# hsiehScalAR/KNODE-Cosserat

Hardware: AMD Instinct MI355X
Metric: rod-steps/sec (N=100 segments, batch=1024) (higher is better)
Workload: dtype f64

## Files before the change

### knode-cosserat_amd/csrc/kr_mso_impl.hpp

```cpp
#pragma once
#include "kr_ms_impl.hpp"

namespace kr {

constexpr int MSO_B0 = 7 + 17 * (MS_P - 1);
#ifndef KR_MSO_LAG
#define KR_MSO_LAG 1
#endif
constexpr int MSO_LAG = KR_MSO_LAG;
static_assert(MSO_B0 + MS_P <= WAVE, "the verifying lanes must fit beside the forward-difference lanes");

template <typename T, int HS>
__host__ __device__ inline size_t mso_lds_elems(int N) {
  return ms_lds_elems<T, HS>(N, true, false) + 80;
}

__device__ __forceinline__ void wave_sync_lds() {
  __builtin_amdgcn_fence(__ATOMIC_ACQ_REL, "wavefront");
  __builtin_amdgcn_wave_barrier();
}

#define KR_LDS __attribute__((address_space(3)))
template <typename T, int NV>
__device__ __forceinline__ void lds_load_vec(const T* src, T (&v)[NV]) {
  using V = typename Vec16<T>::type;
  constexpr int n = Vec16<T>::n;
  static_assert(NV % n == 0, "vector load needs a multiple of 16 bytes");
  const KR_LDS V* s = (const KR_LDS V*)src;
#pragma unroll
  for (int c = 0; c < NV / n; ++c) {
    const V x = s[c];
#pragma unroll
    for (int e = 0; e < n; ++e) v[c * n + e] = x[e];
  }
}
template <typename T, int NV>
__device__ __forceinline__ void lds_store_vec(T* dst, const T (&v)[NV]) {
  using V = typename Vec16<T>::type;
  constexpr int n = Vec16<T>::n;
  static_assert(NV % n == 0, "vector store needs a multiple of 16 bytes");
  KR_LDS V* d = (KR_LDS V*)dst;
#pragma unroll
  for (int c = 0; c < NV / n; ++c) {
    V x;
#pragma unroll
    for (int e = 0; e < n; ++e) x[e] = v[c * n + e];
    d[c] = x;
  }
}

template <typename U>
__device__ __forceinline__ U own_sgpr(U v) {
  asm volatile("" : "+s"(v));
  return v;
}

template <typename U>
__device__ __forceinline__ U* own_sgpr_global(U* p) {
  uintptr_t v = (uintptr_t)p;
  asm volatile("" : "+s"(v));
  return (U*)(__attribute__((address_space(1))) U*)v;
}

#ifdef KR_MS_STAMPS
struct MsoStats { unsigned long long total = 0, sweeps = 0, merged = 0, quick = 0, chord = 0, rejects = 0, retries = 0, rebuilds = 0, t_sweep = 0, t_alg = 0, t_pred = 0, t_verdict = 0, t_cond = 0, t_fin = 0, t_upd = 0, t_v1 = 0, t_v2 = 0, t_c1 = 0, t_c2 = 0, t_copy = 0; };
#endif

template <typename T, bool DIAG, int HS, int OCC = 1, typename PSRC = RodConst<T>>
__global__ __launch_bounds__(WAVE * MS_WPB, OCC) void mso_sim_kernel(const PSRC Pa, const SimArgs<T> A) {
  extern __shared__ __attribute__((aligned(16))) unsigned char smem_raw[];
  const int N = rod_src_N<T>(Pa);
  const int lane = threadIdx.x & (WAVE - 1);
  const int wv = threadIdx.x / WAVE;
  const int64_t rod = (int64_t)blockIdx.x * MS_WPB + wv;
  if (rod >= A.B) return;
  const auto& Pc = rod_src_row<T>(Pa, rod);
  const size_t rod_elems = (size_t)N * KR_SLOTS;
  T* const a_states = own_sgpr_global(A.states);
  const int64_t a_slot_elems = own_sgpr(A.slot_elems);
  const int a_ring = own_sgpr(A.ring);
  T* const a_tip = own_sgpr_global(A.tip);
  int32_t* const a_status = own_sgpr_global(A.status);
  const int a_residual_test = own_sgpr(A.residual_test), a_predictor = own_sgpr(A.predictor);
  const T hc1 = own_sgpr(A.hc1), hc2 = own_sgpr(A.hc2);
  const int T_steps = own_sgpr((int)A.T_steps);
  const MsLds<T> L = ms_carve<T, HS>(reinterpret_cast<T*>(smem_raw) + (size_t)wv * mso_lds_elems<T, HS>(N), N, true, false);
  T* const Es = L.Es;
  T* const XB = L.XB;
  T* const Tm = L.Tm;
  T* const X0 = L.Xs;
  const ptrdiff_t X_d = (L.c12 + (size_t)N * 12) - L.Xs;
  int xsel = 0;
  T* Xs = X0;
  T* XsB = X0 + X_d;
  T* const EsB = Es + MSO_B0 * MS_YP;
  const MsRole R = ms_role(lane, N);
  const int iv = R.iv, col = R.col;
  const bool isA = lane < MSO_B0;
  const bool isB = lane >= MSO_B0 && lane < MSO_B0 + MS_P;
  const int ib = isB ? lane - MSO_B0 : 0;
  const int s_l = isB ? ms_interval_start(ib, R.sbase, R.srem) : R.s_i;
  const int len_l = isB ? R.sbase + (ib < R.srem ? 1 : 0) : R.len_i;
  ms_cold_fill<T>(rod_src_mem<T>(Pa, rod), L.cold, lane);
  wave_sync();

  auto slot_ptr = [&](int slot) -> T* { return a_states + (int64_t)slot * a_slot_elems + rod * rod_elems; };
  auto state_ptr = [&](int k) -> T* { return slot_ptr(a_ring ? k % 3 : k); };
  T* const lead0 = L.c12;
  const ptrdiff_t lead_d = L.hist - L.c12;
  auto lead_of = [&](int t) -> T* { return lead0 + (ptrdiff_t)(t & 1) * lead_d; };
  auto rebuild = [&](int t) {
    const T* cur = state_ptr(t);
    const T* prv = t > 0 ? state_ptr(t - 1) : (A.prev_init ? A.prev_init + rod * rod_elems : cur);
    T* const lc = lead_of(t);
    T* const lp = lead_of(t - 1);
    for (int j = lane; j < N; j += WAVE) {
      T cv[12], pv[12];
      load_hist_vec<T, 12>(cur + (size_t)j * KR_SLOTS, cv);
      load_hist_vec<T, 12>(prv + (size_t)j * KR_SLOTS, pv);
      lds_store_vec<T, 12>(lc + (size_t)j * 12, cv);
      lds_store_vec<T, 12>(lp + (size_t)j * 12, pv);
    }
    wave_sync();
  };
  const T* ctl = A.ctl + rod * A.T_steps * 4;
  auto load_fc = [&](int t) -> V3<T> {
    V3<T> tf{T(0), T(0), T(0)};
#pragma unroll
    for (int k = 0; k < 4; ++k) {
      const T tt = ctl[(size_t)t * 4 + k];
      tf.x += tt * L.cold[CD_TDIRS + k * 3 + 0];
      tf.y += tt * L.cold[CD_TDIRS + k * 3 + 1];
      tf.z += tt * L.cold[CD_TDIRS + k * 3 + 2];
    }
    return {L.cold[CD_RHOAG] + tf.x, L.cold[CD_RHOAG + 1] + tf.y, L.cold[CD_RHOAG + 2] + tf.z};
  };

  const T* s0 = state_ptr(0);
  const T* sp0 = A.prev_init ? A.prev_init + rod * rod_elems : s0;
  MsPred<T> Q;
  double* img = A.pred_io ? A.pred_io + (size_t)rod * MS_PRED_ROWS * WAVE : nullptr;
  if (img && A.pred_load) ms_pred_load<T>(Q, img, lane);
  else ms_pred_init<T>(Q, lane, R, s0, sp0, A.prev_init != nullptr, a_predictor);
  V3<T> vlast, ulast;
  {
    const T* cl = s0 + (size_t)(N - 1) * KR_SLOTS;
    vlast = {cl[SL_V], cl[SL_V + 1], cl[SL_V + 2]};
    ulast = {cl[SL_U], cl[SL_U + 1], cl[SL_U + 2]};
  }
  const T tol = own_sgpr(A.tol), tolA = own_sgpr(A.tolA), fd_eps = own_sgpr(A.fd_eps);
  const int maxit = own_sgpr(A.maxit);
  T kappa = Q.kappa;
  T Gguess = lane < 6 ? A.G[rod * 6 + lane] : T(0);
  MsStamps stamps;
#ifdef KR_MS_STAMPS
  MsoStats st;
  unsigned long long t_begin, tq;
  KR_STAMP(t_begin);
  tq = t_begin;
#endif

  rebuild(0);

  int tA = 0;
  int rsA = 0;
  bool merged = false;
  int it = 0;
  int order = Q.next_order;
  bool retried = false;
  T dn_prev = T(-1);
  bool have_fac = false, below = false;
  float amp = -1.f;
  T dnB = T(-1);
  float ampB = -1.f;
  bool belowB = false;
  int itB = 0, orderB = 0;
  bool pred_skip = false;
  bool reverify = false;
  int resume_at = T_steps;
  T Xreg[MS_P - 1][2];
#pragma unroll
  for (int g = 0; g < MS_P - 1; ++g) Xreg[g][0] = Xreg[g][1] = T(0);
  V3<T> fcA = load_fc(0), fcB = fcA;
  V3<T> fcN = load_fc(T_steps > 1 ? 1 : 0);
  static_assert(DIAG, "the in-sweep history record assumes diagonal material matrices");
  T hk_a[3], hk_b[3], hk_c[3];
#pragma unroll
  for (int c = 0; c < 3; ++c) {
    hk_a[c] = L.cold[CD_KSEI + 4 * c] * L.cold[CD_KSEV + c];
    hk_b[c] = -L.cold[CD_KSEI + 4 * c] * L.cold[CD_BSE + 4 * c];
    hk_c[c] = -L.cold[CD_KBTI + 4 * c] * L.cold[CD_BBT + 4 * c];
  }

  ms_pred_guess<T>(Q, order, lane, L.cold, Xs);
  wave_sync_lds();
  if (order <= 0 && lane < 6) Xs[0 * MS_YP + 7 + lane] = Gguess;
  wave_sync_lds();

  struct Upd { T updP, updG, xsP, xsG, xsY[MS_P - 1]; };

  while (true) {
    const bool runA = tA < T_steps;
    const int tB = tA - 1;
    T yr[19];
    {
      const T* src = isB ? XsB + ib * MS_YP : Xs + iv * MS_YP;
#pragma unroll
      for (int q = 0; q < 19; ++q) yr[q] = src[q];
    }
    const T hstep = (isA && col > 0) ? fd_eps * fmax(fabs(Xs[iv * MS_YP + (R.comp > 0 ? R.comp : 3)]), T(1)) : T(1);
    int comp = R.comp;
    asm volatile("" : "+v"(comp));
#pragma unroll
    for (int q = 3; q < 19; ++q) yr[q] += q == comp ? hstep : T(0);
    RodState<T> y = rows_to_state(yr);
    const V3<T> fc = isB ? fcB : fcA;
    const int lag = (isA && merged) ? MSO_LAG : 0;
    const bool act = isB ? merged : (isA && runA);
    const int trips = R.lmax + ((merged && runA) ? MSO_LAG : 0);
    T* const out_rod = slot_ptr(rsA);
    auto point_of = [&](int k) -> int {
      const int kk = k - lag;
      return s_l + (kk < 0 ? 0 : (kk < len_l ? kk : len_l - 1));
    };
    const T* const lead_n = lead_of(isB ? tB : tA);
    const T* const lead_o = lead_of(isB ? tB + 1 : tB);
    auto hist_older = [&](const T (&lb)[12], T (&pb)[12]) __attribute__((always_inline)) {
#pragma unroll
      for (int c = 0; c < 12; ++c) pb[c] = hc2 * lb[c];
    };
    auto hist_newest = [&](const T (&la)[12], const T (&pb)[12]) __attribute__((always_inline)) -> RodHist<T> {
      T raw[12];
#pragma unroll
      for (int c = 0; c < 12; ++c) raw[c] = fma(hc1, la[c], pb[c]);
      RodHist<T> h;
      h.qh = {raw[0], raw[1], raw[2]};
      h.wh = {raw[3], raw[4], raw[5]};
      h.vh = {raw[6], raw[7], raw[8]};
      h.uh = {raw[9], raw[10], raw[11]};
      h.av = {hk_b[0] * raw[6] + hk_a[0], hk_b[1] * raw[7] + hk_a[1], hk_b[2] * raw[8] + hk_a[2]};
      h.au = {hk_c[0] * raw[9], hk_c[1] * raw[10], hk_c[2] * raw[11]};
      return h;
    };
    auto hist_form = [&](const T (&la)[12], const T (&lb)[12]) __attribute__((always_inline)) -> RodHist<T> {
      T pb[12];
      hist_older(lb, pb);
      return hist_newest(la, pb);
    };
    auto hist_at = [&](int j) __attribute__((always_inline)) -> RodHist<T> {
      T la[12], lb[12];
      lds_load_vec<T, 12>(lead_n + (size_t)j * 12, la);
      lds_load_vec<T, 12>(lead_o + (size_t)j * 12, lb);
      return hist_form(la, lb);
    };
    RodHist<T> hst = hist_at(point_of(0));
    if (!merged) {
      auto fd_point = [&](int j, T dsl) __attribute__((always_inline)) {
        RodState<T> k1;
        V3<T> v, u;
        ode_eval<T, DIAG>(Pc, y, hst, fc, k1, v, u);
        hst = hist_at(j + 1);
        y = state_axpy(y, dsl, k1);
      };
#pragma unroll 2
      for (int t = 0; t < R.sbase; ++t) fd_point(R.s_i + t, Pc.ds);
      if (R.srem) fd_point(R.s_i + (R.len_i > R.sbase ? R.sbase : R.sbase - 1), R.len_i > R.sbase ? Pc.ds : T(0));
    } else {
      const bool lean = a_ring && tB + 4 <= T_steps;
      T* const lead_w = lead_of(tB + 1);
      auto trip = [&](int k, auto full_tag, auto lean_tag) __attribute__((always_inline)) {
        constexpr bool FULL = decltype(full_tag)::value;
        constexpr bool LEAN = decltype(lean_tag)::value;
        const int kk = k - lag;
        const bool live = FULL ? act : (act && kk >= 0 && kk < len_l);
        const int j = FULL ? s_l + kk : point_of(k);
        const int eo = j * 12;
        const int en = FULL ? eo + 12 : point_of(k + 1) * 12;
        T la[12], lb[12], pb[12];
        if constexpr (MSO_LAG >= 2) {
          lds_load_vec<T, 12>(lead_n + en, la);
          lds_load_vec<T, 12>(lead_o + en, lb);
        } else {
          lds_load_vec<T, 12>(lead_o + en, lb);
#ifdef KR_MSO_PROBE_EARLY_READS
          if constexpr (FULL) lds_load_vec<T, 12>(lead_n + en, la);
#endif
        }
        RodState<T> k1;
        V3<T> v, u;
        ode_eval<T, DIAG>(Pc, y, hst, fc, k1, v, u);
        if constexpr (MSO_LAG >= 2) {
          hst = hist_form(la, lb);
          asm volatile("" : "+v"(hst.qh.x), "+v"(hst.qh.y), "+v"(hst.qh.z), "+v"(hst.wh.x), "+v"(hst.wh.y), "+v"(hst.wh.z));
          asm volatile("" : "+v"(hst.vh.x), "+v"(hst.vh.y), "+v"(hst.vh.z), "+v"(hst.uh.x), "+v"(hst.uh.y), "+v"(hst.uh.z));
          asm volatile("" : "+v"(hst.av.x), "+v"(hst.av.y), "+v"(hst.av.z), "+v"(hst.au.x), "+v"(hst.au.y), "+v"(hst.au.z));
        } else {
          hist_older(lb, pb);
          asm volatile("" : "+v"(pb[0]), "+v"(pb[1]), "+v"(pb[2]), "+v"(pb[3]), "+v"(pb[4]), "+v"(pb[5]), "+v"(pb[6]), "+v"(pb[7]),
                            "+v"(pb[8]), "+v"(pb[9]), "+v"(pb[10]), "+v"(pb[11]));
        }
        if (isB && live) {
          T rec[KR_SLOTS];
          record_from(y, v, u, rec);
          T lead[12];
#pragma unroll
          for (int c = 0; c < 12; ++c) lead[c] = rec[c];
          if constexpr (FULL) {
            if constexpr (!LEAN) {
              T rest[KR_SLOTS - 12];
#pragma unroll
              for (int c = 0; c < KR_SLOTS - 12; ++c) rest[c] = rec[12 + c];
              store_vec<T, KR_SLOTS - 12>(out_rod + (size_t)j * KR_SLOTS + 12, rest);
            }
          } else {
            if (!(lean && k >= R.sbase)) store_record(out_rod + (size_t)j * KR_SLOTS, rec);
          }
          lds_store_vec<T, 12>(lead_w + eo, lead);
        }
        if constexpr (MSO_LAG < 2) {
#ifdef KR_MSO_PROBE_EARLY_READS
          if constexpr (!FULL)
#endif
          lds_load_vec<T, 12>(lead_n + en, la);
          if constexpr (OCC == 1) __builtin_amdgcn_sched_barrier(0);
        }
        const T dsl = live ? Pc.ds : T(0);
        y = state_axpy(y, dsl, k1);
        if constexpr (MSO_LAG < 2) {
          asm volatile("" : "+v"(pb[0]), "+v"(pb[1]), "+v"(pb[2]), "+v"(pb[3]), "+v"(pb[4]), "+v"(pb[5]), "+v"(pb[6]), "+v"(pb[7]),
                            "+v"(pb[8]), "+v"(pb[9]), "+v"(pb[10]), "+v"(pb[11]), "+v"(y.p.z), "+v"(y.h3), "+v"(y.n.z), "+v"(y.m.z),
                            "+v"(y.q.z), "+v"(y.w.z));
          hst = hist_newest(la, pb);
        }
      };
      int k = 0;
      for (; k < MSO_LAG && k < trips; ++k) trip(k, std::false_type{}, std::false_type{});
      auto full_trips = [&](auto lean_tag) __attribute__((always_inline)) {
        for (; k + 1 < R.sbase; k += 2) {
          trip(k, std::true_type{}, lean_tag);
          trip(k + 1, std::true_type{}, lean_tag);
        }
        if (k < R.sbase) {
          trip(k, std::true_type{}, lean_tag);
          ++k;
        }
      };
      if (lean) full_trips(std::true_type{});
      else full_trips(std::false_type{});
      for (; k < trips; ++k) trip(k, std::false_type{}, std::false_type{});
    }
#ifdef KR_MS_STAMPS
    KR_STAMP_ADD(st.t_sweep, tq);
    st.sweeps += 1;
    if (merged) st.merged += 1;
#endif

    int ln = lane;
    asm volatile("" : "+v"(ln));
    const int kp = ln & 3;
    const int r = 3 + (ln >> 2);
    const bool plane = ln < 3 * (MS_P - 1);
    const int pi = plane ? ln / 3 : 0;
    const int prow = plane ? ln - 3 * pi : 0;
    const bool glane = ln >= WAVE - 6;
    T er[19];
    state_to_rows(y, er);
    T d[6];
    T updY[MS_P - 1];
    T* dYb = XB;
    float dnf = 0.f;
    bool finite = true;
    Upd U;

    auto finish = [&](const T* X, auto base_slot) -> float {
      T* sp = Tm;
      if (kp == 0) {
#pragma unroll
        for (int g = 1; g < MS_P - 1; ++g) dYb[g * MS_YP + r] = updY[g - 1];
      }
      wave_sync_lds();
      if (plane) {
        const int l0 = pi == 0 ? 0 : 7 + 17 * (pi - 1);
        T s = Es[base_slot(pi) * MS_YP + prow] - X[(pi + 1) * MS_YP + prow];
        T av[16], dv[16];
#pragma unroll
        for (int c = 0; c < 16; ++c) {
          const bool use = pi > 0 || c < 6;
          av[c] = use ? Es[(l0 + 1 + c) * MS_YP + prow] : T(0);
          dv[c] = pi > 0 ? dYb[pi * MS_YP + 3 + c] : T(0);
        }
        __builtin_amdgcn_sched_barrier(0);
        T s2 = T(0);
#pragma unroll
        for (int c = 0; c < 16; c += 2) {
          const T da = pi > 0 ? dv[c] : (c < 6 ? d[c < 6 ? c : 0] : T(0));
          const T db = pi > 0 ? dv[c + 1] : (c + 1 < 6 ? d[c + 1 < 6 ? c + 1 : 0] : T(0));
          s = fma(av[c], da, s);
          s2 = fma(av[c + 1], db, s2);
        }
        sp[pi * 3 + prow] = s + s2;
      }
      wave_sync_lds();
      float nf = 0.f;
      U.updP = T(0); U.updG = T(0); U.xsP = T(0); U.xsG = T(0);
      if (plane) {
        U.xsP = X[(pi + 1) * MS_YP + prow];
#pragma unroll
        for (int i = 0; i < MS_P - 1; ++i) {
          const T t = sp[i * 3 + prow];
          U.updP += i <= pi ? t : T(0);
        }
        nf = update_ratio(U.updP, U.xsP);
      }
      if (glane) {
        const int k = ln - (WAVE - 6);
        U.xsG = X[0 * MS_YP + 7 + k];
        U.updG = k == 0 ? d[0] : k == 1 ? d[1] : k == 2 ? d[2] : k == 3 ? d[3] : k == 4 ? d[4] : d[5];
        nf = fmaxf(nf, update_ratio(U.updG, U.xsG));
      }
#pragma unroll
      for (int g = 1; g < MS_P; ++g) {
        U.xsY[g - 1] = T(0);
        if (((g - 1) & 3) == kp) {
          U.xsY[g - 1] = X[g * MS_YP + r];
          nf = fmaxf(nf, update_ratio(updY[g - 1], U.xsY[g - 1]));
        }
      }
      return wave_max_nonneg(nf);
    };
    auto apply = [&](T* X) {
      if (plane) X[(pi + 1) * MS_YP + prow] = U.xsP + U.updP;
      if (glane) X[0 * MS_YP + 7 + (ln - (WAVE - 6))] = U.xsG + U.updG;
#pragma unroll
      for (int g = 1; g < MS_P; ++g)
        if (((g - 1) & 3) == kp) X[g * MS_YP + r] = U.xsY[g - 1] + updY[g - 1];
    };

    const bool es_stored = merged;
    if (merged) {
      if (isB || (isA && col == 0)) {
#pragma unroll
        for (int q = 0; q < 19; ++q) Es[ln * MS_YP + q] = er[q];
      }
      if (isB) {
        if (ib == MS_P - 1) {
          T rec[KR_SLOTS];
          record_from(y, vlast, ulast, rec);
          store_record(out_rod + (size_t)(N - 1) * KR_SLOTS, rec);
          T lead[12];
#pragma unroll
          for (int c = 0; c < 12; ++c) lead[c] = rec[c];
          lds_store_vec<T, 12>(lead_of(tB + 1) + (size_t)(N - 1) * 12, lead);
          if (a_tip) {
            T* tp = a_tip + (rod * T_steps + tB) * 3;
            tp[0] = y.p.x; tp[1] = y.p.y; tp[2] = y.p.z;
          }
        }
      }
      wave_sync_lds();
#ifdef KR_MS_STAMPS
      unsigned long long tv;
      { KR_STAMP(tv); st.t_v1 += tv - tq; }
#endif
      float rn = 0.f;
      if (ln < 3 * MS_YP) {
        const int g = ln / MS_YP, q = ln - MS_YP * g;
        const T x = XsB[(g + 1) * MS_YP + q];
        rn = update_ratio(EsB[g * MS_YP + q] - x, x);
      } else if (ln < 3 * MS_YP + 6) {
        const int k = ln - 3 * MS_YP;
        const T e = EsB[(MS_P - 1) * MS_YP + 7 + k];
        rn = update_ratio(L.cold[CD_FTIP + k] - e, e);
      }
      rn = wave_max_nonneg(rn);
#ifdef KR_MS_STAMPS
      KR_STAMP_ADD(st.t_v2, tv);
#endif
      const float est = ampB * rn;
      bool accepted = a_residual_test != 0 && ampB > 0.f && T(256) * (T)est <= tol;
      float dnv = est;
#ifdef KR_MS_STAMPS
      if (accepted) st.quick += 1;
#endif
      if (!accepted) {
        T* ach = XB;
        T* rt = XB + 4 * MS_YP;
        dYb = XB + MS_YP * 8;
        T areg[MS_P - 1];
        areg[0] = EsB[0 * MS_YP + r] - XsB[1 * MS_YP + r];
        if (kp == 0) ach[1 * MS_YP + r] = areg[0];
        wave_sync_lds();
#pragma unroll
        for (int g = 1; g < MS_P; ++g) {
          const int l0 = 7 + 17 * (g - 1);
          T av[4], xv[4];
#pragma unroll
          for (int cc = 0; cc < 4; ++cc) {
            av[cc] = Es[(l0 + 1 + 4 * kp + cc) * MS_YP + r];
            xv[cc] = ach[g * MS_YP + 3 + 4 * kp + cc];
          }
          const T e0 = EsB[g * MS_YP + r];
          const T ynext = g < MS_P - 1 ? XsB[(g + 1) * MS_YP + r] : T(0);
          T part = fma(av[0], xv[0], av[1] * xv[1]) + fma(av[2], xv[2], av[3] * xv[3]);
          part += quad_xor<0xB1>(part);
          part += quad_xor<0x4E>(part);
          if (g < MS_P - 1) {
            areg[g] = e0 - ynext + part;
            if (kp == 0) ach[(g + 1) * MS_YP + r] = areg[g];
          } else if (kp == 0 && r >= 7 && r < 13) {
            rt[r - 7] = L.cold[CD_FTIP + (r - 7)] - e0 - part;
          }
          wave_sync_lds();
        }
        {
          T rtv[6];
#pragma unroll
          for (int j = 0; j < 6; ++j) rtv[j] = rt[j];
#pragma unroll
          for (int i = 0; i < 6; ++i) {
            T acc = T(0);
#pragma unroll
            for (int j = 0; j < 6; ++j) acc = fma(L.Ti[i * 6 + j], rtv[j], acc);
            d[i] = acc;
          }
        }
        {
          const T dd0 = kp == 0 ? T(0) : kp == 1 ? d[1] : kp == 2 ? d[3] : d[5];
          const T dd1 = kp == 0 ? d[0] : kp == 1 ? d[2] : kp == 2 ? d[4] : T(0);
#pragma unroll
          for (int g = 1; g < MS_P; ++g) {
            T sx = fma(Xreg[g - 1][1], dd1, Xreg[g - 1][0] * dd0);
            sx += quad_xor<0xB1>(sx);
            sx += quad_xor<0x4E>(sx);
            updY[g - 1] = areg[g - 1] + sx;
          }
        }
        dnv = finish(XsB, [](int g) { return MSO_B0 + g; });
        accepted = dnv <= 3.0e38f && (T)dnv <= T(0.5) * tol;
#ifdef KR_MS_STAMPS
        st.chord += 1;
#endif
      }
      if (accepted) {
        {
          const T* const lt = lead_of(tB + 1);
          for (int j = ln; j < N; j += WAVE) {
            T lv[12];
            lds_load_vec<T, 12>(lt + (size_t)j * 12, lv);
            store_vec<T, 12>(out_rod + (size_t)j * KR_SLOTS, lv);
          }
        }
        if (!belowB && dnB > T(0)) {
          const T floor_dn = T(64) * (sizeof(T) == 8 ? T(2.2e-16) : T(1.2e-7));
          const T kq = fmax((T)dnv, floor_dn) * fast_rcp(dnB * dnB);
          kappa = fmin(fmax(kq, T(1e-4)), T(1));
        }
        if (ln == 0 && a_status) a_status[rod * T_steps + tB] = KR_ST_CONVERGED;
        if (ln < 6) Gguess = XsB[0 * MS_YP + 7 + ln];
        pred_skip = false;
        reverify = false;
        merged = false;
        if (!runA) break;
      } else {
#ifdef KR_MS_STAMPS
        st.rejects += 1;
#endif
        const bool ok = dnv <= 3.0e38f;
        if (ok) apply(XsB);
        wave_sync_lds();
        if (ok && !reverify && itB + 2 <= maxit) {
          reverify = true;
          itB += 1;
          dnB = (T)dnv;
          __builtin_amdgcn_fence(__ATOMIC_ACQ_REL, "agent");
          rebuild(tB);
#ifdef KR_MS_STAMPS
          st.rebuilds += 1;
          KR_STAMP_ADD(st.t_alg, tq);
#endif
          continue;
        }
        reverify = false;
        for (int e = ln; e < MS_NE; e += WAVE) Xs[e] = XsB[e];
        tA = tB;
        rsA = a_ring ? (rsA == 0 ? 2 : rsA - 1) : rsA - 1;
        fcN = fcA;
        fcA = fcB;
        order = orderB;
        it = itB;
        dn_prev = ok ? (T)dnv : T(-1);
        have_fac = ok;
        amp = ampB;
        below = false;
        pred_skip = true;
        merged = false;
        __builtin_amdgcn_fence(__ATOMIC_ACQ_REL, "agent");
        rebuild(tA);
#ifdef KR_MS_STAMPS
        st.rebuilds += 1;
        KR_STAMP_ADD(st.t_alg, tq);
#endif
        if (it >= maxit) { resume_at = tA; break; }
        continue;
      }
    }

#ifdef KR_MS_STAMPS
    { unsigned long long t_; KR_STAMP(t_); st.t_verdict += t_ - tq; }
    unsigned long long tq2;
    KR_STAMP(tq2);
#endif
    ++it;
    float res_full;
    {
      const int l0own = iv == 0 ? 0 : 7 + 17 * (iv - 1);
      if (!es_stored) {
        if (isA && col == 0) {
#pragma unroll
          for (int q = 0; q < 19; ++q) Es[ln * MS_YP + q] = er[q];
        }
        wave_sync_lds();
      }
      res_full = ms_residual_norm<T>(Es, Xs, L.cold, ln);
      if (isA && col > 0) {
        const T ih = fast_rcp(hstep);
        T e0[19];
#pragma unroll
        for (int q = 0; q < 19; ++q) e0[q] = Es[l0own * MS_YP + q];
        __builtin_amdgcn_sched_barrier(0);
#pragma unroll
        for (int q = 0; q < 19; ++q) Es[ln * MS_YP + q] = (er[q] - e0[q]) * ih;
      }
      wave_sync_lds();
    }
#ifdef KR_MS_STAMPS
    unsigned long long tc;
    { KR_STAMP(tc); st.t_c1 += tc - tq2; }
#endif
    dYb = XB;
    {
      const T c0 = Es[0 * MS_YP + r] - Xs[1 * MS_YP + r];
      const T da = Es[(2 * kp) * MS_YP + r];
      const T db = Es[(2 * kp + 1) * MS_YP + r];
      Xreg[0][0] = kp == 0 ? c0 : da;
      Xreg[0][1] = kp == 3 ? T(0) : db;
      store_pair(XB + r * 8 + 2 * kp, Xreg[0][0], Xreg[0][1]);
    }
    wave_sync_lds();
#pragma unroll
    for (int g = 1; g < MS_P; ++g) {
      const T* xcur = XB + ((g - 1) & 1) * (MS_YP * 8);
      T* xnext = XB + (g & 1) * (MS_YP * 8);
      const int l0 = 7 + 17 * (g - 1);
      const T e0 = Es[l0 * MS_YP + r];
      T n0 = T(0), n1 = T(0), n2 = T(0), n3 = T(0);
      if (g < MS_P - 1) {
        const T cg = e0 - Xs[(g + 1) * MS_YP + r];
        n0 = kp == 0 ? cg : T(0);
      }
      {
        T av[16], xa[16], xb[16];
#pragma unroll
        for (int c = 0; c < 16; ++c) {
          av[c] = Es[(l0 + 1 + c) * MS_YP + r];
          load_pair(xcur + (3 + c) * 8 + 2 * kp, xa[c], xb[c]);
        }
        __builtin_amdgcn_sched_barrier(0);
#pragma unroll
        for (int c = 0; c < 16; c += 2) {
          n0 = fma(av[c], xa[c], n0);
          n1 = fma(av[c], xb[c], n1);
          n2 = fma(av[c + 1], xa[c + 1], n2);
          n3 = fma(av[c + 1], xb[c + 1], n3);
        }
        n0 += n2;
        n1 += n3;
      }
      if (g < MS_P - 1) {
        Xreg[g][0] = n0;
        Xreg[g][1] = n1;
        store_pair(xnext + r * 8 + 2 * kp, n0, n1);
      } else if (r >= 7 && r < 13) {
        if (kp == 0) n0 = L.cold[CD_FTIP + (r - 7)] - e0 - n0;
        store_pair(Tm + (r - 7) * 8 + 2 * kp, n0, n1);
      }
      wave_sync_lds();
    }
#ifdef KR_MS_STAMPS
    KR_STAMP_ADD(st.t_c2, tc);
#endif
    {
      T a6[6][7];
      auto fill6 = [&](T (&m)[6][7]) {
#pragma unroll
        for (int i = 0; i < 6; ++i) {
          T row[8];
          load_hist_vec<T, 8>(Tm + i * 8, row);
#pragma unroll
          for (int k = 0; k < 6; ++k) m[i][k] = row[1 + k];
          m[i][6] = ln < 6 ? (ln == i ? T(1) : T(0)) : row[0];
        }
      };
      fill6(a6);
      T x6[6];
      solve6_uniform(a6, x6, fill6);
      if (ln < 6) {
#pragma unroll
        for (int i = 0; i < 6; ++i) L.Ti[i * 6 + ln] = x6[i];
      }
#pragma unroll
      for (int i = 0; i < 6; ++i) d[i] = lane_bcast<6>(x6[i]);
      have_fac = true;
    }
    {
      const T dd0 = kp == 0 ? T(1) : kp == 1 ? d[1] : kp == 2 ? d[3] : d[5];
      const T dd1 = kp == 0 ? d[0] : kp == 1 ? d[2] : kp == 2 ? d[4] : T(0);
#pragma unroll
      for (int g = 1; g < MS_P; ++g) {
        T s = fma(Xreg[g - 1][1], dd1, Xreg[g - 1][0] * dd0);
        s += quad_xor<0xB1>(s);
        s += quad_xor<0x4E>(s);
        updY[g - 1] = s;
      }
    }
#ifdef KR_MS_STAMPS
    KR_STAMP_ADD(st.t_cond, tq2);
#endif
    dnf = finish(Xs, [](int g) { return g == 0 ? 0 : 7 + 17 * (g - 1); });
#ifdef KR_MS_STAMPS
    KR_STAMP_ADD(st.t_fin, tq2);
#endif
    finite = dnf <= 3.0e38f;
    const T dn = (T)dnf;
    if (res_full > 0.f && finite) amp = dnf / res_full;
    if (finite && !below && dn <= tol) {
      below = true;
      if (dn_prev > T(0)) {
        const T floor_dn = T(64) * (sizeof(T) == 8 ? T(2.2e-16) : T(1.2e-7));
        const T kq = fmax(dn, floor_dn) * fast_rcp(dn_prev * dn_prev);
        kappa = fmin(fmax(kq, T(1e-4)), T(1));
      }
    }
    bool next_final = false;
    if (finite) {
      apply(Xs);
      next_final = predict_final<T>(dn, dn_prev, tol, tolA) || (kappa > T(0) && T(4) * kappa * dn * dn <= tol);
      dn_prev = dn;
    }
    wave_sync_lds();
#ifdef KR_MS_STAMPS
    KR_STAMP_ADD(st.t_alg, tq);
#endif
    if (!finite || (it >= maxit && !(next_final && dn <= T(1e-2)))) {
      if (order > 0 && !retried) {
        retried = true;
        order = 0;
        ms_pred_guess<T>(Q, 0, ln, L.cold, Xs);
        wave_sync_lds();
        if (ln < 6) Xs[0 * MS_YP + 7 + ln] = Gguess;
        wave_sync_lds();
        it = 0; dn_prev = T(-1); have_fac = false; amp = -1.f; below = false;
#ifdef KR_MS_STAMPS
        st.retries += 1;
#endif
        continue;
      }
      resume_at = tA;
      break;
    }
    if (next_final && dn <= T(1e-2)) {
      xsel ^= 1;
      Xs = X0 + xsel * X_d;
      XsB = X0 + (1 - xsel) * X_d;
#ifdef KR_MS_STAMPS
      { unsigned long long t_; KR_STAMP(t_); st.t_copy += t_ - tq; }
#endif
      dnB = dn; ampB = amp; belowB = below; itB = it; orderB = order;
      if (!pred_skip) ms_pred_update<T>(Q, order, KR_ST_CONVERGED, a_predictor, lane, XsB, stamps);
#ifdef KR_MS_STAMPS
      { unsigned long long t_; KR_STAMP(t_); st.t_upd += t_ - tq; }
#endif
      tA += 1;
      rsA = a_ring ? (rsA == 2 ? 0 : rsA + 1) : rsA + 1;
      fcB = fcA;
      if (tA < T_steps) {
        fcA = fcN;
        fcN = load_fc(tA + 1 < T_steps ? tA + 1 : tA);
        order = Q.next_order;
        ms_pred_guess<T>(Q, order, lane, L.cold, Xs);
        wave_sync_lds();
        if (order <= 0 && lane < 6) Xs[0 * MS_YP + 7 + lane] = XsB[0 * MS_YP + 7 + lane];
        wave_sync_lds();
      }
      it = 0; retried = false; below = false; dn_prev = T(-1);
      merged = true;
#ifdef KR_MS_STAMPS
      KR_STAMP_ADD(st.t_pred, tq);
#endif
    }
  }

  if (lane < 6) A.G[rod * 6 + lane] = Gguess;
  if (lane == 0 && A.resume) A.resume[rod] = (int32_t)resume_at;
  if (img && (resume_at >= T_steps || !A.resume)) {
    Q.kappa = kappa;
    ms_pred_save<T>(Q, img, lane);
  }
#ifdef KR_MS_STAMPS
  if (lane == 0 && A.dbg) {
    unsigned long long te;
    KR_STAMP(te);
    unsigned long long* dd = A.dbg + rod * 24;
    dd[0] = te - t_begin; dd[1] = st.t_sweep; dd[2] = st.t_alg; dd[3] = st.t_pred; dd[4] = st.sweeps;
    dd[5] = st.merged; dd[6] = st.quick; dd[7] = st.chord; dd[8] = st.rejects; dd[9] = st.retries; dd[10] = st.rebuilds;
    dd[11] = (unsigned long long)resume_at;
    dd[12] = st.t_verdict; dd[13] = st.t_cond; dd[14] = st.t_fin; dd[15] = st.t_upd;
    dd[16] = stamps.a1; dd[17] = stamps.a2; dd[18] = stamps.a3; dd[19] = st.t_v1; dd[20] = st.t_v2; dd[21] = st.t_c1; dd[22] = st.t_c2; dd[23] = st.t_copy;
  }
#endif
}

template <typename T, int OCC, typename PSRC>
static int launch_mso_inst(const PSRC& P, const SimPlan& p, const SimArgs<T>& a, const LaunchAt& at) {
  return launch(at, mso_sim_kernel<T, true, hs_phys<T>(), OCC, PSRC>, dim3((unsigned)((a.B + MS_WPB - 1) / MS_WPB)), dim3(WAVE * MS_WPB),
                p.smem[0], P, a);
}
template <typename T>
int launch_mso_sim(kr_handle* h, const SimPlan& p, const SimArgs<T>& a, const LaunchAt& at) {
  if constexpr (sizeof(T) == 4) {
    if (p.occ == 2) return launch_mso_inst<T, 2>(consts<T>(h), p, a, at);
  }
  return launch_mso_inst<T, 1>(consts<T>(h), p, a, at);
}

}
```

Baseline: 46.22 million.

## Specialize predictor update for LP fits and skip redundant tip record stores

Adds a specialized predictor-update path, used when OCC==1, for when the last order was the LP predictor and its fit is good. It evaluates only the LP fit error and refits only when the fit is stale or fails the threshold, instead of running the general multi-order update. It also skips writing the tip record to global memory while in lean ring mode, where later steps overwrite it. The risks are that a kept LP fit becomes a worse predictor and costs more Newton iterations, and that lean mode may drop a tip record some consumer still needs.

```diff
diff --git a/knode-cosserat_amd/csrc/kr_mso_impl.hpp b/knode-cosserat_amd/csrc/kr_mso_impl.hpp
--- a/knode-cosserat_amd/csrc/kr_mso_impl.hpp
+++ b/knode-cosserat_amd/csrc/kr_mso_impl.hpp
@@ -60,6 +60,83 @@
   uintptr_t v = (uintptr_t)p;
   asm volatile("" : "+s"(v));
   return (U*)(__attribute__((address_space(1))) U*)v;
+}
+
+template <typename T, int NC>
+__device__ __forceinline__ void mso_pred_update(MsPred<T, NC>& Q, int order, int predictor, int lane, const T* Xs,
+                                                MsStamps& stamps) {
+  if (!__builtin_amdgcn_readfirstlane((int)(order == MS_ORDER_LP && Q.lp_good))) {
+    ms_pred_update<T>(Q, order, KR_ST_CONVERGED, predictor, lane, Xs, stamps);
+    return;
+  }
+#ifdef KR_MS_STAMPS
+  unsigned long long tpu;
+  KR_STAMP(tpu);
+#endif
+  float err_lp = 0.f;
+  if (Q.lp_have) {
+#pragma unroll
+    for (int q = 0; q < MS_EPL; ++q) {
+      const int e = lane + q * WAVE;
+      if (e < MS_NE) {
+        const double x = (double)Xs[e];
+        double b[NC];
+        lp_basis<T, NC>(Q.Hx[q], b);
+        err_lp = fmaxf(err_lp, update_ratio(x - lp_eval<NC>(Q.lpa, b), x));
+      }
+    }
+  }
+  const float em_lp = wave_max_nonneg(err_lp);
+#ifdef KR_MS_STAMPS
+  KR_STAMP_ADD(stamps.a1, tpu);
+#endif
+  const bool lp_tested = Q.lp_have;
+  const bool keep_fit = lp_tested && em_lp < 1.0e-3f && Q.lp_age < 3;
+  Q.lp_age = keep_fit ? Q.lp_age + 1 : 0;
+  Q.lp_have = keep_fit;
+  if (!keep_fit && predictor >= MS_ORDER_LP && Q.avail >= NC - 1) {
+    double Sn[lp_nsum<NC>()];
+#pragma unroll
+    for (int k = 0; k < lp_nsum<NC>(); ++k) Sn[k] = 0.0;
+#pragma unroll
+    for (int q = 0; q < MS_EPL; ++q) {
+      const int e = lane + q * WAVE;
+      if (e < MS_NE) {
+        const double x = (double)Xs[e];
+        double b[NC];
+        lp_basis<T, NC>(Q.Hx[q], b);
+        const double w = (double)__builtin_amdgcn_rcpf(fmaxf(fabsf((float)x), 1.0f));
+        lp_accumulate<NC>(Sn, b, x, w);
+      }
+    }
+#pragma unroll
+    for (int k = 0; k < lp_nsum<NC>(); ++k) Sn[k] = wave_sum_f64(Sn[k]);
+    double a[NC];
+    if (lp_solve<NC>(Sn, a)) {
+#pragma unroll
+      for (int k = 0; k < NC; ++k) Q.lpa[k] = a[k];
+      Q.lp_have = true;
+    }
+  }
+#ifdef KR_MS_STAMPS
+  KR_STAMP_ADD(stamps.a2, tpu);
+#endif
+  Q.next_order = Q.avail < predictor ? Q.avail : (predictor < MS_HLEV ? predictor : MS_HLEV - 1);
+  Q.lp_good = lp_tested && Q.lp_have && em_lp < 1.0e-3f;
+  if (lp_tested && Q.lp_have && (em_lp < 3.0e38f || Q.lp_good)) Q.next_order = MS_ORDER_LP;
+#ifdef KR_MS_STAMPS
+  stamps.osum += (unsigned long long)order; stamps.olast = order;
+  for (int p = 0; p < MS_HLEV; ++p) stamps.em[p] = 3.0e38f;
+  KR_STAMP_ADD(stamps.a3, tpu);
+#endif
+#pragma unroll
+  for (int q = 0; q < MS_EPL; ++q) {
+    const int e = lane + q * WAVE;
+#pragma unroll
+    for (int k = MS_HLEV - 1; k > 0; --k) Q.Hx[q][k] = Q.Hx[q][k - 1];
+    if (e < MS_NE) Q.Hx[q][0] = Xs[e];
+  }
+  if (Q.avail < MS_HLEV - 1) ++Q.avail;
 }
 
 #ifdef KR_MS_STAMPS
@@ -254,6 +331,7 @@
       return hist_form(la, lb);
     };
     RodHist<T> hst = hist_at(point_of(0));
+    const bool lean = a_ring && tB + 4 <= T_steps;
     if (!merged) {
       auto fd_point = [&](int j, T dsl) __attribute__((always_inline)) {
         RodState<T> k1;
@@ -266,7 +344,6 @@
       for (int t = 0; t < R.sbase; ++t) fd_point(R.s_i + t, Pc.ds);
       if (R.srem) fd_point(R.s_i + (R.len_i > R.sbase ? R.sbase : R.sbase - 1), R.len_i > R.sbase ? Pc.ds : T(0));
     } else {
-      const bool lean = a_ring && tB + 4 <= T_steps;
       T* const lead_w = lead_of(tB + 1);
       auto trip = [&](int k, auto full_tag, auto lean_tag) __attribute__((always_inline)) {
         constexpr bool FULL = decltype(full_tag)::value;
@@ -446,7 +523,7 @@
         if (ib == MS_P - 1) {
           T rec[KR_SLOTS];
           record_from(y, vlast, ulast, rec);
-          store_record(out_rod + (size_t)(N - 1) * KR_SLOTS, rec);
+          if (!lean) store_record(out_rod + (size_t)(N - 1) * KR_SLOTS, rec);
           T lead[12];
 #pragma unroll
           for (int c = 0; c < 12; ++c) lead[c] = rec[c];
@@ -776,7 +853,10 @@
       { unsigned long long t_; KR_STAMP(t_); st.t_copy += t_ - tq; }
 #endif
       dnB = dn; ampB = amp; belowB = below; itB = it; orderB = order;
-      if (!pred_skip) ms_pred_update<T>(Q, order, KR_ST_CONVERGED, a_predictor, lane, XsB, stamps);
+      if (!pred_skip) {
+        if constexpr (OCC == 1) mso_pred_update<T>(Q, order, a_predictor, lane, XsB, stamps);
+        else ms_pred_update<T>(Q, order, KR_ST_CONVERGED, a_predictor, lane, XsB, stamps);
+      }
 #ifdef KR_MS_STAMPS
       { unsigned long long t_; KR_STAMP(t_); st.t_upd += t_ - tq; }
 #endif
```

New measurement: 46.83 million (median of 6 runs). 1.01x the previous value.
